# svohr/mixemt

Hardware: AMD Instinct MI355X
Metric: read x hap cells/sec through the EM iteration (EM iters/sec reported beside it as em_iters_per_s), 1000000 reads x 5408 haps in total, whole job (higher is better)
Workload: dtype f64

## Files before the change

include/mixemt_hip_tuning.h:

```cpp
#ifndef MIXEMT_HIP_TUNING_H
#define MIXEMT_HIP_TUNING_H

#include <stddef.h>
#include <stdint.h>

#ifdef __cplusplus
extern "C" {
#endif

struct mxm_em_state;

int mxm_reset_tuning(void);

int mxm_set_timing_events(void *ev_start, void *ev_stop);

int mxm_describe_stream_kernel(int32_t H, int32_t nb, char *buf, size_t len);

int mxm_diag_stream_read(const void *src, size_t bytes, int32_t wg_per_cu, int32_t blocked,
                         void *sink, void *stream);

struct mxm_coded;
int mxm_diag_stream_coded(const struct mxm_coded *c, int32_t H, int32_t wg_per_cu, void *sink, void *stream);

int mxm_diag_stream_quads(const struct mxm_coded *c, int32_t H, int32_t wg_per_cu, void *sink, void *stream);

int mxm_set_progress_callback(void (*fn)(const struct mxm_em_state *state_host, int32_t B, void *user),
                              void *user, int32_t every);

int mxm_set_loop_graph(int32_t mode);

int mxm_set_loop_fused(int32_t mode, int32_t chunk);

int mxm_set_fused_coded_grid(int32_t nwg);

int mxm_set_quad_left_grid(int32_t nwg);

int mxm_set_sparse_long_rows(int32_t on);
int mxm_set_sparse_long_entries(int32_t n);

int mxm_set_quad_encoder(int32_t kind);

int mxm_set_coded_batch_tile(int32_t bt);

int mxm_diag_fused_force_abort(int32_t on);

int mxm_diag_fused_stamps(const void *ws, unsigned long long *out_host);

int mxm_set_batch_tile(int32_t bt);

int mxm_set_compact_restarts(int32_t mode);

#define MXM_SAMPLES_TILE_ROWS 32
int mxm_samples_tile_rows(void);

int mxm_set_min_rows_per_wg(int32_t n);

int mxm_set_sparse_max_distinct(int32_t n);

#ifdef __cplusplus
}
#endif
#endif
```

mixemt_amd/_lib.py:

```python

import ctypes
import os

_PKG = os.path.dirname(os.path.abspath(__file__))
LIB_PATH = os.environ.get("MXM_LIB") or os.path.join(_PKG, "lib", "libmixemt_hip.so")

c_i32, c_i64, c_f64 = ctypes.c_int32, ctypes.c_int64, ctypes.c_double
c_ptr, c_size = ctypes.c_void_p, ctypes.c_size_t


class EmState(ctypes.Structure):
    _fields_ = [("done", c_i32), ("iters", c_i32), ("l1", c_f64), ("ticket", ctypes.c_uint32), ("error", ctypes.c_uint32)]


class Coded(ctypes.Structure):
    _fields_ = [("rec", c_ptr), ("rec_off", c_ptr), ("ndist", c_ptr), ("R", c_i64),
                ("P_rest", c_ptr), ("ldp_rest", c_i64), ("w_rest", c_ptr), ("R_rest", c_i64),
                ("wide_rows", c_ptr), ("n_wide", c_i64),
                ("qrec", c_ptr), ("qoff", c_ptr), ("nquad", c_ptr), ("quad_rows", c_ptr), ("n_quad_rows", c_i64),
                ("byte_rows", c_ptr), ("n_byte_rows", c_i64)]


class SampleTile(ctypes.Structure):
    _fields_ = [("sample", c_i32), ("count", c_i32), ("first", c_i64)]
# ... 80 lines not shown
                                         ctypes.POINTER(EmState)]),
    "mxm_samples_tile_rows": (ctypes.c_int, []),
    "mxm_samples_plan": (c_i64, [c_ptr, c_i32, c_ptr, c_i64, c_ptr]),
    "mxm_samples_workspace_bytes": (c_size, [c_i64, c_i32, c_i32]),
    "mxm_em_iter_samples": (ctypes.c_int, [ctypes.POINTER(Coded), c_ptr, c_i32, c_ptr, c_ptr, c_i32, c_ptr, c_ptr, c_ptr,
                                           c_size, c_ptr]),
    "mxm_em_loop_samples": (ctypes.c_int, [ctypes.POINTER(Coded), c_ptr, c_i32, c_ptr, c_i32, c_ptr, c_ptr, c_ptr, c_ptr,
                                           c_ptr, c_f64, c_i32, c_i32, c_ptr, c_size, c_ptr, ctypes.POINTER(EmState)]),
    "mxm_em_step": (ctypes.c_int, [c_ptr, c_i64, c_ptr, c_ptr, c_i64, c_i32, c_ptr, c_i64, c_i32,
                                   c_ptr, c_ptr, c_size, c_ptr]),
    "mxm_log_normalize": (ctypes.c_int, [c_ptr, c_i32, c_ptr, c_ptr]),
    "mxm_l1_exp_diff": (ctypes.c_int, [c_ptr, c_ptr, c_i32, c_ptr, c_ptr]),
    "mxm_add_scalar": (ctypes.c_int, [c_ptr, c_i64, c_i64, c_i32, c_f64, c_ptr]),
    "mxm_assign_reads": (ctypes.c_int, [c_ptr, c_i64, c_ptr, c_ptr, c_i32, c_i64, c_i32, c_f64, c_ptr, c_ptr]),
    "mxm_diag_stream_read": (ctypes.c_int, [c_ptr, c_size, c_i32, c_i32, c_ptr, c_ptr]),
    "mxm_diag_stream_coded": (ctypes.c_int, [ctypes.POINTER(Coded), c_i32, c_i32, c_ptr, c_ptr]),
    "mxm_diag_stream_quads": (ctypes.c_int, [ctypes.POINTER(Coded), c_i32, c_i32, c_ptr, c_ptr]),
    "mxm_diag_fused_force_abort": (ctypes.c_int, [c_i32]),
    "mxm_set_fused_coded_grid": (ctypes.c_int, [c_i32]),
    "mxm_set_quad_left_grid": (ctypes.c_int, [c_i32]),
    "mxm_set_coded_batch_tile": (ctypes.c_int, [c_i32]),
    "mxm_set_sparse_long_rows": (ctypes.c_int, [c_i32]),
    "mxm_set_quad_encoder": (ctypes.c_int, [c_i32]),
    "mxm_set_sparse_long_entries": (ctypes.c_int, [c_i32]),
    "mxm_diag_fused_stamps": (ctypes.c_int, [c_ptr, ctypes.POINTER(ctypes.c_ulonglong)]),
    "mxm_set_timing_events": (ctypes.c_int, [c_ptr, c_ptr]),
    "mxm_set_batch_tile": (ctypes.c_int, [c_i32]),
    "mxm_encode_signatures": (ctypes.c_int64, [ctypes.c_char_p, c_ptr, c_i64, c_ptr, c_i64, c_ptr, c_ptr, c_ptr,
                                               c_i64]),
    "mxm_aln_encode": (ctypes.c_int, [ctypes.POINTER(AlnColumns), c_ptr, c_i64, c_ptr, c_i32, c_i32, c_i32, c_i32,
                                      ctypes.POINTER(c_ptr)]),
    "mxm_aln_sizes_of": (ctypes.c_int, [c_ptr, ctypes.POINTER(AlnSizes)]),
    "mxm_aln_fetch": (ctypes.c_int, [c_ptr, c_ptr, c_ptr, c_ptr, c_ptr, c_ptr, c_ptr, c_ptr, c_ptr, c_ptr]),
    "mxm_aln_fetch_fragments": (ctypes.c_int, [c_ptr, c_ptr, c_ptr, c_ptr, c_ptr]),
    "mxm_aln_free": (None, [c_ptr]),
    "mxm_bam_read": (ctypes.c_int, [ctypes.c_char_p, c_i32, ctypes.POINTER(c_ptr)]),
    "mxm_bam_sizes_of": (ctypes.c_int, [c_ptr, ctypes.POINTER(BamSizes)]),
    "mxm_bam_columns": (ctypes.c_int, [c_ptr, ctypes.POINTER(AlnColumns)]),
    "mxm_bam_fetch_names": (ctypes.c_int, [c_ptr, c_ptr, c_ptr, c_ptr, c_ptr]),
    "mxm_bam_free": (None, [c_ptr]),
    "mxm_observe_bases": (ctypes.c_int, [ctypes.POINTER(AlnColumns), c_ptr, c_i32, c_i32, c_i64, c_ptr, c_ptr]),
    "mxm_observe_bases_labelled": (ctypes.c_int, [ctypes.POINTER(AlnColumns), c_ptr, c_ptr, c_i32, c_i32, c_i32, c_i64,
                                                  c_ptr, c_ptr]),
    "mxm_consensus": (ctypes.c_int, [c_ptr, c_i32, c_i64, c_i64, c_i64, c_i32, c_ptr, c_ptr, c_ptr, c_ptr]),
    "mxm_new_variants": (ctypes.c_int, [c_ptr, c_i64, c_i32, ctypes.POINTER(c_i32), c_i32, c_i64, c_ptr, c_ptr, c_ptr]),
    "mxm_first_observed": (ctypes.c_int, [ctypes.POINTER(AlnColumns), c_ptr, c_ptr, c_i32, c_i32, c_i32, c_i64, c_ptr,
                                          c_ptr, c_ptr]),
    "mxm_extend_assign": (ctypes.c_int, [ctypes.POINTER(AlnColumns), c_ptr, c_ptr, c_i32, c_i32, ctypes.POINTER(c_i32),
                                         c_i32, c_i32, c_i32, c_i32, c_ptr, c_i64, c_ptr, c_ptr, c_ptr, c_ptr]),
    "mxm_set_compact_restarts": (ctypes.c_int, [c_i32]),
    "mxm_set_loop_graph": (ctypes.c_int, [c_i32]),
    "mxm_set_loop_fused": (ctypes.c_int, [c_i32, c_i32]),
    "mxm_set_progress_callback": (ctypes.c_int, [c_ptr, c_ptr, c_i32]),
    "mxm_set_min_rows_per_wg": (ctypes.c_int, [c_i32]),
    "mxm_reset_tuning": (ctypes.c_int, []),
    "mxm_describe_stream_kernel": (ctypes.c_int, [c_i32, c_i32, ctypes.c_char_p, c_size]),
    "mxm_set_sparse_max_distinct": (ctypes.c_int, [c_i32]),
    "mxm_row_argmax_votes": (ctypes.c_int, [c_ptr, c_i64, c_ptr, c_i64, c_i32, c_ptr, c_ptr,
                                            c_ptr, c_size, c_ptr]),
    "mxm_first_seen": (ctypes.c_int, [c_ptr, c_i64, c_i32, c_ptr, c_ptr]),
    "mxm_gather_columns": (ctypes.c_int, [c_ptr, c_i64, c_i64, c_i32, c_ptr, c_i32, c_ptr, c_i64, c_ptr]),
    "mxm_fold_logaddexp": (ctypes.c_int, [c_ptr, c_i64, ctypes.POINTER(c_ptr), ctypes.POINTER(c_i64), c_i32,
                                          c_i64, c_i32, c_f64, c_ptr]),
}

FINISH_SIGNATURES = {
    "mxm_samples_finish_workspace_bytes": (c_size, [c_i64, c_i32, c_i32]),
    "mxm_votes_samples": (ctypes.c_int, [ctypes.POINTER(Coded), c_ptr, c_i32, c_i32, c_ptr, c_ptr, c_ptr, c_ptr, c_ptr, c_ptr,
                                         c_ptr, c_ptr, c_ptr, c_ptr, c_ptr, c_size, c_ptr]),
    "mxm_gather_columns_samples": (ctypes.c_int, [ctypes.POINTER(Coded), c_ptr, c_i32, c_i32, c_ptr, c_ptr, c_i32, c_ptr,
                                                  c_ptr, c_size, c_ptr]),
    "mxm_em_loop_samples_narrow": (ctypes.c_int, [ctypes.POINTER(Coded), c_ptr, c_i32, c_i32, c_ptr, c_i32, c_ptr, c_ptr,
                                                  c_ptr, c_ptr, c_ptr, c_ptr, c_f64, c_i32, c_i32, c_ptr, c_ptr, c_size,
                                                  c_ptr, ctypes.POINTER(EmState)]),
    "mxm_assign_reads_samples": (ctypes.c_int, [ctypes.POINTER(Coded), c_ptr, c_i32, c_i32, c_ptr, c_i32, c_ptr, c_ptr,
                                                c_ptr, c_ptr, c_ptr, c_ptr, c_f64, c_ptr, c_ptr, c_ptr, c_size, c_ptr]),
}

VARCHECK_SIGNATURES = {
    "mxm_check_variants_samples": (ctypes.c_int, [c_ptr, c_i32, c_i64, c_ptr, c_ptr, c_i32, c_ptr, c_ptr, c_i32, c_i64, c_ptr,
                                                  c_ptr, c_i32, c_f64, c_f64, c_f64, c_i32, c_i32, c_ptr, c_ptr, c_ptr, c_ptr]),
}

ABI_VERSION = 603

PROGRESS_FN = ctypes.CFUNCTYPE(None, ctypes.POINTER(EmState), c_i32, c_ptr)

_lib = None


class MixemtHipError(RuntimeError):
    pass


def load():
    global _lib
    if _lib is not None:
        return _lib
    if not os.path.exists(LIB_PATH):
        raise MixemtHipError(
            "libmixemt_hip.so is not built (%s); run `python -m mixemt_amd.build` -- "
            "there is no CPU fallback for the EM hot path" % LIB_PATH)
    from . import _dev
    lib = ctypes.CDLL(LIB_PATH)
    try:
        lib.mxm_version.restype = ctypes.c_int
        lib.mxm_version.argtypes = []
        have = lib.mxm_version()
    except AttributeError:
        have = None
    if have != ABI_VERSION:
        raise MixemtHipError("%s reports ABI version %s, this binding was written for %d: rebuild with "
                             "`python -m mixemt_amd.build --force`" % (LIB_PATH, have, ABI_VERSION))
    for name, (restype, argtypes) in (list(SIGNATURES.items()) + list(FINISH_SIGNATURES.items())
                                      + list(VARCHECK_SIGNATURES.items())):
        try:
            fn = getattr(lib, name)
        except AttributeError:
            raise MixemtHipError("%s has ABI version %d but lacks %s: rebuild with "
                                 "`python -m mixemt_amd.build --force`" % (LIB_PATH, have, name))
        fn.restype = restype
        fn.argtypes = argtypes
    _lib = lib
    try:
        if _dev.torch is not None and _dev.torch.cuda.is_available():
            lib.mxm_preload()
    except Exception:
        pass
    return lib


def check(rc, what):
    if rc != 0:
        msg = load().mxm_last_error().decode("utf-8", "replace")
        raise ValueError("%s failed (%d): %s" % (what, rc, msg))
```

mixemt_amd/build.py:

```python

import hashlib
import os
import shutil
import subprocess
import sys

_PKG = os.path.dirname(os.path.abspath(__file__))
_ROOT = os.path.dirname(_PKG)
SRC = os.path.join(_PKG, "csrc", "mixemt_hip.hip")
HDRS = [os.path.join(_ROOT, "include", name) for name in ("mixemt_hip.h", "mixemt_hip_tuning.h", "mixemt_hip_samples_finish.h",
                                                           "mixemt_hip_var_check.h")]
LIB_DIR = os.path.join(_PKG, "lib")
LIB = os.path.join(LIB_DIR, "libmixemt_hip.so")
ARCH = "gfx950"


def _hipcc():
    for cand in (os.environ.get("HIPCC"), shutil.which("hipcc"), "/opt/rocm/bin/hipcc"):
        if cand and os.path.exists(cand):
            return cand
    raise RuntimeError("hipcc not found (set HIPCC or add /opt/rocm/bin to PATH)")


def _sources():
    csrc = os.path.dirname(SRC)
    return sorted(os.path.join(csrc, f) for f in os.listdir(csrc) if f.endswith((".hip", ".hpp"))) + HDRS


def _digest(flags):
    h = hashlib.sha256()
    for path in _sources():
        with open(path, "rb") as fin:
            h.update(fin.read())
    h.update(" ".join(flags).encode())
    return h.hexdigest()


def build(force=False, defines=(), verbose=False, out=None):
    global LIB
    if out is not None:
        LIB = os.path.abspath(out)
    flags = ["--offload-arch=%s" % ARCH, "-O3", "-std=c++17", "-shared", "-fPIC", "-Werror=format",
             "-I" + os.path.join(_ROOT, "include"), "-I" + os.path.dirname(SRC)]
    flags += ["-D%s" % d for d in defines]
    stamp = LIB + ".stamp"
    want = _digest(flags)
    if not force and os.path.exists(LIB) and os.path.exists(stamp):
        with open(stamp) as fin:
            if fin.read().strip() == want:
                return LIB
    os.makedirs(os.path.dirname(LIB), exist_ok=True)
    cmd = [_hipcc()] + flags + [SRC, "-o", LIB, "-lz"]
    if verbose:
        sys.stderr.write(" ".join(cmd) + "\n")
    proc = subprocess.run(cmd, stdout=subprocess.PIPE, stderr=subprocess.STDOUT, text=True)
    if proc.returncode != 0:
        raise RuntimeError("hipcc failed:\n" + proc.stdout)
    with open(stamp, "w") as fout:
        fout.write(want + "\n")
    return LIB


if __name__ == "__main__":
    defs = []
    argv = sys.argv[1:]
    i = 0
    while i < len(argv):
        if argv[i] == "-D":
            defs.append(argv[i + 1])
            i += 2
        elif argv[i].startswith("-D"):
            defs.append(argv[i][2:])
            i += 1
        else:
            i += 1
    out_path = argv[argv.index("--out") + 1] if "--out" in argv else None
    print(build(force="--force" in argv, defines=defs, verbose=True, out=out_path))
```

mixemt_amd/csrc/coded_kernels.hpp:

```cpp
#ifndef MIXEMT_CODED_KERNELS_HPP
#define MIXEMT_CODED_KERNELS_HPP

#define ENC_THREADS 256
#define ENC_SLOTS 1024
#define ENC_MAX_CODES 256
#define ENC_MAX_WIDE 1024
#define ENC_WIDE_SLOTS 4096
#define ENC_EMPTY 0xFFFFFFFFFFFFFFFFull

__host__ __device__ __forceinline__ int rec_code_bytes(int nd, int ldc) { return nd > ENC_MAX_CODES ? 2 * ldc : ldc; }
__device__ __forceinline__ int rec_code_at(const uint8_t *codes, int h, bool wide) {
    return wide ? (int)reinterpret_cast<const uint16_t *>(codes)[h] : (int)codes[h];
}

template <int NCH, bool WIDE>
__device__ __forceinline__ void encode_one_row(int64_t r, const double *__restrict__ M, int64_t ldm, int H, int ldc,
                                               uint8_t *__restrict__ rec, int64_t rec_cap, int64_t *__restrict__ rec_off,
                                               int32_t *__restrict__ ndist, double *__restrict__ rowmax,
                                               unsigned long long *__restrict__ stats) {
    constexpr int NW = ENC_THREADS / 64;
    constexpr int SLOTS = WIDE ? ENC_WIDE_SLOTS : ENC_SLOTS;
    constexpr int MAXC = WIDE ? ENC_MAX_WIDE : ENC_MAX_CODES;
    constexpr int SPT = SLOTS / ENC_THREADS;
    __shared__ unsigned long long s_key[SLOTS];
// ... 89 lines not shown
            }
        }
    }
    __syncthreads();
    const bool dense = (s_flag != 0);

    int cnt = 0;
#pragma unroll
    for (int j = 0; j < SPT; ++j) cnt += (s_key[SPT * t + j] != ENC_EMPTY) ? 1 : 0;
    const int incl = wave_inclusive_scan_i32(cnt);
    if (lane == 63) s_wcnt[wv] = incl;
    __syncthreads();
    int base = 0, D = 0;
#pragma unroll
    for (int q = 0; q < NW; ++q) {
        if (q < wv) base += s_wcnt[q];
        D += s_wcnt[q];
    }
    const int cbytes = WIDE ? 2 * ldc : ldc;
    const int64_t bytes = (int64_t)cbytes + 16 * (int64_t)D;
    const bool coded = !dense && D <= MAXC && (!WIDE || D > ENC_MAX_CODES);
    if (t == 0) {
        long long off = -1;
        if (coded) {
            off = (long long)atomicAdd(&stats[0], (unsigned long long)bytes);
            if (off + bytes > rec_cap) off = -1;
        }
        s_off = off;
    }
    int code = base + incl - cnt;
#pragma unroll
    for (int j = 0; j < SPT; ++j) {
        if (s_key[SPT * t + j] != ENC_EMPTY) s_code[SPT * t + j] = (unsigned short)code++;
    }
    __syncthreads();
    const long long off = s_off;
    if (off >= 0) {
        double *tbl = reinterpret_cast<double *>(rec + off + cbytes);
        code = base + incl - cnt;
#pragma unroll
        for (int j = 0; j < SPT; ++j) {
            const unsigned long long kk = s_key[SPT * t + j];
            if (kk != ENC_EMPTY) {
                const double mval = __longlong_as_double((long long)kk);
                tbl[code] = exp(mval - shift);
                tbl[D + code] = mval;
                ++code;
            }
        }
#pragma unroll
        for (int k = 0; k < NCH; ++k) {
            const int c0 = 4 * (t + k * ENC_THREADS);
            if (c0 < ldc) {
                unsigned int cd[4];
#pragma unroll
                for (int e = 0; e < 4; ++e) cd[e] = (c0 + e < H) ? (unsigned int)s_code[slot[k][e]] : 0u;
                if constexpr (WIDE) {
                    u2 word;
                    word.x = cd[0] | (cd[1] << 16);
                    word.y = cd[2] | (cd[3] << 16);
                    reinterpret_cast<u2 *>(rec + off)[t + k * ENC_THREADS] = word;
                } else {
                    reinterpret_cast<unsigned int *>(rec + off)[t + k * ENC_THREADS] =
                        cd[0] | (cd[1] << 8) | (cd[2] << 16) | (cd[3] << 24);
                }
            }
        }
    }
    if (t == 0) {
        if constexpr (WIDE) {
            if (off >= 0) {
                ndist[r] = D;
                rec_off[r] = off;
                atomicAdd(&stats[1], ~0ull);
            }
        } else {
            rowmax[r] = shift;
            ndist[r] = (off >= 0) ? D : 0;
            rec_off[r] = (off >= 0) ? off : 0;
            if (off < 0) atomicAdd(&stats[1], 1ull);
        }
    }
    __syncthreads();
}

template <int NCH>
__global__ __launch_bounds__(ENC_THREADS) void encode_rows_kernel(
    const double *__restrict__ M, int64_t ldm, int64_t R, int H, int ldc, uint8_t *__restrict__ rec, int64_t rec_cap,
    int64_t *__restrict__ rec_off, int32_t *__restrict__ ndist, double *__restrict__ rowmax,
    unsigned long long *__restrict__ stats) {
    for (int64_t r = blockIdx.x; r < R; r += gridDim.x)
        encode_one_row<NCH, false>(r, M, ldm, H, ldc, rec, rec_cap, rec_off, ndist, rowmax, stats);
}

template <int NCH>
__global__ __launch_bounds__(ENC_THREADS) void encode_wide_rows_kernel(
    const double *__restrict__ M, int64_t ldm, int64_t R, int H, int ldc, uint8_t *__restrict__ rec, int64_t rec_cap,
    int64_t *__restrict__ rec_off, int32_t *__restrict__ ndist, double *__restrict__ rowmax,
    unsigned long long *__restrict__ stats) {
    constexpr int CH = 32;
    __shared__ int s_list[CH];
    __shared__ int s_nlist;
    const int t = threadIdx.x;
    const int64_t nchunk = (R + CH - 1) / CH;
    for (int64_t c = blockIdx.x; c < nchunk; c += gridDim.x) {
        if (t == 0) s_nlist = 0;
        __syncthreads();
        const int64_t r = c * CH + t;
        if (t < CH && r < R && ndist[r] == 0) s_list[atomicAdd(&s_nlist, 1)] = t;
        __syncthreads();
        const int n = s_nlist;
        for (int i = 0; i < n; ++i)
            encode_one_row<NCH, true>(c * CH + s_list[i], M, ldm, H, ldc, rec, rec_cap, rec_off, ndist, rowmax, stats);
        __syncthreads();
    }
}

template <int THREADS, int NCH, int NBUF, bool NT, bool RESIDENT, bool WIDE_PREFETCH, bool CHECK = false>
__device__ __forceinline__ void coded_row_pass(const uint8_t *__restrict__ rec, const int64_t *__restrict__ rec_off,
                                               const int32_t *__restrict__ ndist, int ldc, const double *__restrict__ w,
                                               const int64_t *__restrict__ wide_rows, int64_t n_wide, int64_t R,
                                               const double (&p)[NCH][4], double (&acc)[NCH][4], bool &meta_ready,
                                               int *chk_result = nullptr, const int64_t *__restrict__ row_list = nullptr,
                                               int64_t n_list = 0, const int32_t *__restrict__ nquad = nullptr, int vbid = -1,
                                               int vgrid = 0) {
    static_assert(NBUF >= 3, "codes NBUF - 1 rows ahead, tables NBUF - 2");
    constexpr int NW = THREADS / 64;
    constexpr int AUX = NT ? 2 : 0;
    __shared__ double s_tbl[NBUF][ENC_MAX_CODES];
    __shared__ __attribute__((aligned(16))) double red[NBUF][NW];
    const int t = threadIdx.x, lane = t & 63, wv = t >> 6;
    const int nword = ldc >> 2;
    const int64_t bid = vbid >= 0 ? (int64_t)vbid : (int64_t)blockIdx.x, grid = vbid >= 0 ? (int64_t)vgrid : (int64_t)gridDim.x;
    const row_deal deal(row_list != nullptr ? n_list : R, bid, grid);
    const int voff = t * 4;
    int last_w = t + (NCH - 1) * THREADS;
    if (last_w > nword - 1) last_w = nword - 1;
    const int voff_last = last_w * 4;
    const bool tbl_thread = (THREADS <= ENC_MAX_CODES) || t < ENC_MAX_CODES;
    const int tslot = t & (ENC_MAX_CODES - 1);
    typedef unsigned int u2v __attribute__((ext_vector_type(2)));
    __shared__ int s_chk[2];
    if constexpr (CHECK) {
        if (t == 0) s_chk[0] = s_chk[1] = 0;
        __syncthreads();
    }
    auto list_row = [&](int64_t e) -> int64_t {
        int64_t r = wide_rows[e];
        if constexpr (CHECK) {
            if (r < 0 || r >= R || (e > 0 && wide_rows[e - 1] >= r)) {
                s_chk[1] = 1;
                r = -1;
            }
        }
        return r;
    };
    auto list_nd = [&](int64_t r) -> int {
        if (r < 0) return 0;
        int nd = ndist[r];
        if constexpr (CHECK) {
            if (nd <= ENC_MAX_CODES) {
                s_chk[1] = 1;
                nd = 0;
            }
        }
        return nd;
// ... 444 lines not shown
```

mixemt_amd/csrc/mixemt_hip.hip:

```cpp
#include <hip/hip_runtime.h>
#include <stdint.h>
#include <stdio.h>
#include <stdlib.h>
#include <string.h>
#include <math.h>
#include <algorithm>
#include <atomic>
#include <mutex>
#include <type_traits>
#include <utility>
#include <vector>

#include "mixemt_hip.h"
#include "mixemt_hip_tuning.h"

#include "common.hpp"
#include "aln_encode.hpp"
#include "bam_reader.hpp"
#include "coded_kernels.hpp"
#include "quad_kernels.hpp"
#include "quad_batched_kernels.hpp"
#include "build_kernels.hpp"
#include "build_lut_kernels.hpp"
#include "build_sparse_kernels.hpp"
#include "em_kernels.hpp"
#include "estep_kernels.hpp"
#include "aux_kernels.hpp"
#include "records_kernels.hpp"
#include "fused_kernels.hpp"
#include "fused_cols_kernels.hpp"
#include "fused_coded_kernels.hpp"
#include "fused_narrow_kernels.hpp"
#include "samples_kernels.hpp"
#include "samples_finish_kernels.hpp"
#include "exchange.hpp"
#include "aln_walk.hpp"
#include "observe_kernels.hpp"
#include "var_check_kernels.hpp"
#include "assemble_kernels.hpp"


struct mxm_em_state;
typedef void (*mxm_progress_fn)(const mxm_em_state *state_host, int32_t B, void *user);
struct mxm_tuning {
    int sparse_maxd = -1;
    int min_rows_per_wg = 8;
    int compact_restarts = 2;
    int max_bt = 4;
    int loop_graph = -1;
    int loop_fused = -1;
    int fused_chunk = 0;
    int fused_cols = 1;
    int fused_coded_wg = 0;
    int quad_left_wg = 0;
    int sparse_long_entries = 5120;
    int quad_encoder = 1;
    int sparse_long = 1;
    int coded_bt = 3;
    int fused_force_abort = 0;
    double fused_cells = 1.0e8;
    hipEvent_t ev_start = nullptr, ev_stop = nullptr;
    mxm_progress_fn progress = nullptr;
    void *progress_user = nullptr;
    int progress_every = 10;
};
static std::mutex g_tune_mu;
static mxm_tuning g_tune;
static thread_local mxm_tuning T;
#define MXM_ENTER() do { std::lock_guard<std::mutex> lk_(g_tune_mu); T = g_tune; } while (0)
template <typename F>
static int tune_set(F f) {
    std::lock_guard<std::mutex> lk(g_tune_mu);
    f(g_tune);
    return 0;
}
extern "C" int mxm_reset_tuning(void) {
    return tune_set([](mxm_tuning &t) { t = mxm_tuning(); });
}

static inline int clamp_grid(int64_t want, int cap) {
    if (want < 1) want = 1;
    return (int)(want < cap ? want : cap);
}

static inline int64_t part_ld(int H) { return ((int64_t)H + 1) & ~(int64_t)1; }

static hipError_t raise_dynamic_lds(const void *kernel, size_t bytes, const char *name) {
    const hipError_t e = hipFuncSetAttribute(kernel, hipFuncAttributeMaxDynamicSharedMemorySize, (int)bytes);
    if (e != hipSuccess)
        snprintf(g_err, sizeof(g_err), "%s: cannot opt into %zu bytes of dynamic LDS: %s", name, bytes,
                 hipGetErrorString(e));
    return e;
}
static int dynamic_lds_ok(const void *kernel, size_t bytes, const char *name, const char *who = nullptr, int H = 0,
                          const char *too_wide = nullptr) {
    if (too_wide != nullptr && bytes > 150 * 1024) return fail(-1, "%s: H=%d %s", who, H, too_wide);
    if (bytes > 60 * 1024 && raise_dynamic_lds(kernel, bytes, name) != hipSuccess) return -2;
    return 0;
}

#define RC_TRY(expr)                                                                         \
    do {                                                                                     \
        const int rc_ = (expr);                                                              \
        if (rc_ != 0) return rc_;                                                            \
    } while (0)

template <int MAX, typename F>
static bool dispatch_width(int n, F &&f) {
    if constexpr (MAX < 1) {
        return false;
    } else {
        if (n != MAX) return dispatch_width<MAX - 1>(n, f);
        f(std::integral_constant<int, MAX>{});
        return true;
    }
}

extern "C" int mxm_version(void) { return MXM_VERSION; }
extern "C" const char *mxm_last_error(void) { return g_err; }

extern "C" int mxm_linear_supported(int32_t H) {
    return (H >= MXM_LINEAR_MIN_H && H <= 8192) ? 1 : 0;
}

static size_t fused_sync_bytes() { return (sizeof(fused_sync) + 255) & ~(size_t)255; }
static size_t fused_snapshot_bytes(int H, int B) {
    return ((size_t)3 * B * H * sizeof(double) + (size_t)B * sizeof(mxm_em_state) + 255) & ~(size_t)255;
}
static size_t fused_rows_bytes(int H, int nwg) { return (size_t)(nwg + 2) * part_ld(H) * sizeof(double); }
static size_t fused_cols_bytes(int64_t R, int nwg) {
    const size_t ldz = (size_t)((R + 1) & ~(int64_t)1);
    return ((size_t)(nwg + 1) * ldz + 2 * (size_t)nwg) * sizeof(double);
}

extern "C" size_t mxm_workspace_bytes(int64_t R, int32_t H, int32_t B) {
    const size_t tiles = (size_t)MXM_MAX_WG * MXM_MAX_BT * (size_t)part_ld(H) * sizeof(double);
    size_t fused = fused_rows_bytes(H, MXM_MAX_WG);
    if (R > 0 && R <= (int64_t)FCOLS_MAX_RPT * FCOLS_THREADS) fused = std::max(fused, fused_cols_bytes(R, MXM_MAX_WG));
    fused += fused_sync_bytes() + fused_snapshot_bytes(H, B > 0 ? B : 1) + 512;
// ... 226 lines not shown
        rec_off == nullptr || ndist == nullptr || rowmax == nullptr || stats == nullptr)
        return fail(-1, "mxm_build_em_records: record buffer (16-byte aligned, >= one record) and output arrays required");
    spb_records out;
    out.rec = rec;
    out.rec_cap = (long long)rec_bytes;
    out.rec_off = rec_off;
    out.ndist = ndist;
    out.rowmax = rowmax;
    out.stats = reinterpret_cast<unsigned long long *>(stats);
    out.ldc = coded_ld(H);
    return build_sparse_impl("mxm_build_em_records", maj, lhit, lmiss, mk_ptr, mk_hap, mk_base, row_ptr, site, obs, order,
                             R, H, S, M, ldm, &out, fallback, n_fallback, (hipStream_t)stream);
}

template <typename ST>
static int linearize_wide(const double *M, int64_t ldm, int64_t R, int H, ST *P, int64_t ldp, double *rowmax,
                          hipStream_t s) {
    const int nch = (H / 2 + 255) / 256;
    int cap = num_cu() * 2 < MXM_MAX_WG ? num_cu() * 2 : MXM_MAX_WG;
    const int nwg = clamp_grid((R + 1) / 2, cap);
    const bool ok = dispatch_width<16>(nch, [&](auto n) {
        hipLaunchKernelGGL((linearize_wide_kernel<decltype(n)::value, ST>), dim3(nwg), dim3(256), 0, s, M, ldm, R, H, P, ldp, rowmax);
    });
    return ok ? 0 : 1;
}

static inline bool wide_rows_ok(const void *M, int64_t ldm, int H) {
    return ((H & 1) == 0) && ((ldm & 1) == 0) && ((reinterpret_cast<uintptr_t>(M) & 15) == 0) && H >= 64 && H <= 8192;
}

extern "C" int mxm_linearize(const double *M, int64_t ldm, int64_t R, int32_t H, double *P, int64_t ldp,
                             double *rowmax, void *stream) {
    if (R < 0 || H <= 0) return fail(-1, "mxm_linearize: bad shape");
    if (ldm < H || ldp < H || (ldp & 1)) return fail(-1, "mxm_linearize: ldp must be even and >= H (ldp=%lld)", (long long)ldp);
    if (R == 0) return 0;
    if (wide_rows_ok(M, ldm, H) && (reinterpret_cast<uintptr_t>(P) & 15) == 0 &&
        linearize_wide<double>(M, ldm, R, (int)H, P, ldp, rowmax, (hipStream_t)stream) == 0) {
        HIP_TRY(hipGetLastError());
        return 0;
    }
    const int grid = clamp_grid(R, num_cu() * 8);
    hipLaunchKernelGGL(linearize_kernel, dim3(grid), dim3(ROW_THREADS), 0, (hipStream_t)stream, M, ldm, R,
                       (int)H, P, ldp, rowmax);
    HIP_TRY(hipGetLastError());
    return 0;
}

extern "C" int mxm_set_timing_events(void *ev_start, void *ev_stop) {
    return tune_set([=](mxm_tuning &t) { t.ev_start = (hipEvent_t)ev_start; t.ev_stop = (hipEvent_t)ev_stop; });
}

extern "C" int mxm_set_min_rows_per_wg(int32_t n) {
    if (n < 1) return fail(-1, "mxm_set_min_rows_per_wg: n < 1");
    return tune_set([n](mxm_tuning &t) { t.min_rows_per_wg = n; });
}

extern "C" int mxm_set_compact_restarts(int32_t mode) {
    return tune_set([mode](mxm_tuning &t) { t.compact_restarts = mode < 0 ? 0 : (mode > 2 ? 2 : mode); });
}

extern "C" int mxm_set_batch_tile(int32_t bt) {
    if (bt < 1 || bt > 4) return fail(-1, "mxm_set_batch_tile: tile must be 1..4");
    return tune_set([bt](mxm_tuning &t) { t.max_bt = bt; });
}

extern "C" int mxm_set_fused_coded_grid(int32_t nwg) {
    return tune_set([nwg](mxm_tuning &t) { t.fused_coded_wg = nwg > 0 ? nwg : 0; });
}

extern "C" int mxm_set_sparse_long_rows(int32_t on) {
    return tune_set([on](mxm_tuning &t) { t.sparse_long = on ? 1 : 0; });
}
extern "C" int mxm_set_sparse_long_entries(int32_t n) {
    return tune_set([n](mxm_tuning &t) { t.sparse_long_entries = n > 0 ? n : 0; });
}
extern "C" int mxm_set_coded_batch_tile(int32_t bt) {
    if (bt != 1 && bt != 3) return fail(-1, "mxm_set_coded_batch_tile: 1 or 3, got %d", bt);
    return tune_set([bt](mxm_tuning &t) { t.coded_bt = bt; });
}
extern "C" int mxm_set_quad_encoder(int32_t kind) {
    if (kind != 0 && kind != 1) return fail(-1, "mxm_set_quad_encoder: 0 or 1, got %d", kind);
    return tune_set([kind](mxm_tuning &t) { t.quad_encoder = kind; });
}
extern "C" int mxm_set_quad_left_grid(int32_t nwg) {
    return tune_set([nwg](mxm_tuning &t) { t.quad_left_wg = nwg > 0 ? nwg : 0; });
}

extern "C" int mxm_diag_fused_force_abort(int32_t on) {
    return tune_set([on](mxm_tuning &t) { t.fused_force_abort = on ? 1 : 0; });
}

#ifndef MXM_V1_THREADS
#define MXM_V1_THREADS 256
#endif
#ifndef MXM_V1_NBUF
#define MXM_V1_NBUF 2
#endif
#ifndef MXM_V1_WG_PER_CU
#define MXM_V1_WG_PER_CU 2
#endif
#ifndef MXM_V2_THREADS
#define MXM_V2_THREADS 512
#endif
#ifndef MXM_V2_NBUF
#define MXM_V2_NBUF 2
#endif
#ifndef MXM_V3_THREADS
#define MXM_V3_THREADS 512
#endif
#ifndef MXM_V3_NBUF
#define MXM_V3_NBUF 2
#endif
#ifndef MXM_V4_THREADS
#define MXM_V4_THREADS 512
#endif
#ifndef MXM_V4_NBUF
#define MXM_V4_NBUF 2
#endif
#ifndef MXM_V2_PREG
#define MXM_V2_PREG 1
#endif
#ifndef MXM_V3_PREG
#define MXM_V3_PREG 2
#endif
#ifndef MXM_V4_PREG
#define MXM_V4_PREG 2
#endif
#ifndef MXM_V1B_THREADS
#define MXM_V1B_THREADS 512
#endif
#ifndef MXM_V1B_NBUF
#define MXM_V1B_NBUF 3
#endif
#define MXM_MAX_COL2 4096
#define MXM_LDS_BUDGET (156 * 1024)

static inline int variant_threads(int nb) {
    return nb == 1 ? MXM_V1_THREADS : (nb == 2 ? MXM_V2_THREADS : (nb == 3 ? MXM_V3_THREADS : MXM_V4_THREADS));
}
static inline int variant_preg(int nb) {
    return nb == 1 ? 1 : (nb == 2 ? MXM_V2_PREG : (nb == 3 ? MXM_V3_PREG : MXM_V4_PREG));
}

static size_t batch_lds_bytes(int H, int nb) {
    const int threads = variant_threads(nb);
    const int nch = ((H + 1) / 2 + threads - 1) / threads;
    return (size_t)(nb - variant_preg(nb)) * nch * threads * 16;
}

static bool batch_fits(int H, int nb) {
    if (nb <= 1) return true;
    static const int max_nch[MXM_MAX_BT + 1] = {0, 16, 8, 7, 6};
    const int threads = variant_threads(nb);
    const int nch = ((H + 1) / 2 + threads - 1) / threads;
    return nch <= max_nch[nb] && batch_lds_bytes(H, nb) <= MXM_LDS_BUDGET;
}

template <int THREADS, int NCH, int BT, int NBUF, int PREG>
static int launch_wide(const double *P, int64_t ldp, const double *w, const double *props, int64_t R,
                       int H, int grid, double *partial, int64_t ldpart,
                       const mxm_em_state *state, mxm_slots slots, hipStream_t stream) {
    if constexpr (NCH * THREADS > MXM_MAX_COL2) {
        return fail(-1, "mxm_em_iter: H=%d outside the linear kernel's range", H);
    } else {
        const size_t lds = (size_t)(BT - PREG) * NCH * THREADS * sizeof(d2);
        RC_TRY(dynamic_lds_ok(reinterpret_cast<const void *>(&em_iter_wide_kernel<THREADS, NCH, BT, NBUF, PREG>), lds, "em_iter_wide_kernel"));
// ... 180 lines not shown
        hipLaunchKernelGGL((estep_global_kernel<true>), dim3(nwg), dim3(ROW_THREADS), 0, stream, M, ldm, w, ln_props, R, H,
                           (double *)nullptr, (int64_t)0, 0, partial, ldpart, state, (const int64_t *)nullptr);
        HIP_TRY(hipGetLastError());
    } else if (H <= MXM_NARROW_MAX_H) {
        const int rc = launch_narrow<true>(M, ldm, w, ln_props, R, H, (double *)nullptr, (int64_t)0, 0, partial, ldpart,
                                           state, stream, &nwg);
        if (rc != 0) return rc;
    } else {
        nwg = clamp_grid(R, num_cu() * 2 < MXM_MAX_WG ? num_cu() * 2 : MXM_MAX_WG);
        RC_TRY(dynamic_lds_ok(reinterpret_cast<const void *>(&estep_log_kernel<true>), lds, "estep_log_kernel"));
        hipLaunchKernelGGL((estep_log_kernel<true>), dim3(nwg), dim3(ROW_THREADS), lds, stream, M, ldm, w, ln_props,
                           R, H, (double *)nullptr, (int64_t)0, 0, partial, ldpart, state);
        HIP_TRY(hipGetLastError());
    }
    return reduce_one(partial, nwg, H, colsum, state, stream);
}

extern "C" int mxm_em_iter(const double *M, int64_t ldm, const double *P, int64_t ldp, const double *w,
                           const double *props, const double *ln_props, int64_t R, int32_t H, int32_t B,
                           const mxm_em_state *state, double *colsum, void *ws, size_t ws_bytes, void *stream) {
    MXM_ENTER();
    if (R <= 0 || H <= 0 || B <= 0) return fail(-1, "mxm_em_iter: bad shape R=%lld H=%d", (long long)R, H);
    if (ws == nullptr || ws_bytes < mxm_workspace_bytes(R, H, B)) return fail(-1, "mxm_em_iter: workspace too small");
    if (P != nullptr && ((ldp & 1) || ldp < H)) return fail(-1, "mxm_em_iter: ldp must be even and >= H");
    if (M != nullptr && ldm < H) return fail(-1, "mxm_em_iter: ldm < H");
    const bool linear = (P != nullptr) && mxm_linear_supported(H);
    int max_bt = linear ? T.max_bt : 1;
    while (max_bt > 1 && !batch_fits((int)H, max_bt)) --max_bt;
    for (int b = 0; b < B;) {
        const int left = B - b;
        const int passes = (left + max_bt - 1) / max_bt;
        const int nb = (left + passes - 1) / passes;
        const mxm_em_state *st = state ? state + b : nullptr;
        int rc;
        if (linear)
            rc = em_iter_linear_tile(P, ldp, w, props, R, (int)H, nb, slots_from(b), state, colsum, (double *)ws,
                                     (hipStream_t)stream, b == 0);
        else
            rc = em_iter_log_one(M, ldm, w, ln_props ? ln_props + (int64_t)b * H : nullptr, R, (int)H, st,
                                 colsum + (int64_t)b * H, (double *)ws, (hipStream_t)stream);
        if (rc != 0) return rc;
        b += nb;
    }
    return 0;
}

extern "C" int mxm_linearize_f32(const double *M, int64_t ldm, int64_t R, int32_t H, float *P, int64_t ldp,
                                 double *rowmax, void *stream) {
    if (R < 0 || H <= 0) return fail(-1, "mxm_linearize_f32: bad shape");
    if (ldm < H || ldp < H || (ldp & 3)) return fail(-1, "mxm_linearize_f32: ldp must be a multiple of 4 and >= H (ldp=%lld)", (long long)ldp);
    if (R == 0) return 0;
    if (wide_rows_ok(M, ldm, H) && (reinterpret_cast<uintptr_t>(P) & 7) == 0 && (ldp & 1) == 0 &&
        linearize_wide<float>(M, ldm, R, (int)H, P, ldp, rowmax, (hipStream_t)stream) == 0) {
        HIP_TRY(hipGetLastError());
        return 0;
    }
    const int grid = clamp_grid(R, num_cu() * 8);
    hipLaunchKernelGGL(linearize_f32_kernel, dim3(grid), dim3(ROW_THREADS), 0, (hipStream_t)stream, M, ldm, R, (int)H,
                       P, ldp, rowmax);
    HIP_TRY(hipGetLastError());
    return 0;
}

extern "C" int mxm_em_iter_f32(const float *P, int64_t ldp, const double *w, const double *props, int64_t R,
                               int32_t H, int32_t B, const mxm_em_state *state, double *colsum, void *ws,
                               size_t ws_bytes, void *stream) {
    MXM_ENTER();
    if (R <= 0 || H <= 0 || B <= 0) return fail(-1, "mxm_em_iter_f32: bad shape R=%lld H=%d", (long long)R, H);
    if (!mxm_linear_supported(H)) return fail(-1, "mxm_em_iter_f32: H=%d outside the linear kernel's range", H);
    if (P == nullptr || (ldp & 3) || ldp < H) return fail(-1, "mxm_em_iter_f32: ldp must be a multiple of 4 and >= H");
    if (ws == nullptr || ws_bytes < mxm_workspace_bytes(R, H, B)) return fail(-1, "mxm_em_iter_f32: workspace too small");
    for (int b = 0; b < B; ++b) {
        const int rc = em_iter_f32_one(P, ldp, w, props + (int64_t)b * H, R, (int)H, state ? state + b : nullptr,
                                       colsum + (int64_t)b * H, (double *)ws, (hipStream_t)stream, b == 0);
        if (rc != 0) return rc;
    }
    return 0;
}

extern "C" size_t mxm_coded_bytes(int64_t R, int32_t H) { return mxm_record_bytes(R, H); }

extern "C" int mxm_encode_rows(const double *M, int64_t ldm, int64_t R, int32_t H, uint8_t *rec, size_t rec_bytes,
                               int64_t *rec_off, int32_t *ndist, double *rowmax, int64_t *stats, void *stream) {
    if (R <= 0 || H <= 0 || ldm < H) return fail(-1, "mxm_encode_rows: bad shape R=%lld H=%d", (long long)R, H);
    if (!mxm_linear_supported(H) || (reinterpret_cast<uintptr_t>(M) & 7) != 0)
        return fail(-1, "mxm_encode_rows: needs H in [65, 8192] (H=%d ldm=%lld)", H, (long long)ldm);
    if (rec == nullptr || (reinterpret_cast<uintptr_t>(rec) & 15) || rec_bytes < (size_t)coded_ld(H) + 16 * ENC_MAX_CODES)
        return fail(-1, "mxm_encode_rows: record buffer missing, unaligned or smaller than one record");
    if (rec_off == nullptr || ndist == nullptr || rowmax == nullptr || stats == nullptr)
        return fail(-1, "mxm_encode_rows: output arrays required");
    hipStream_t s = (hipStream_t)stream;
    HIP_TRY(hipMemsetAsync(stats, 0, 2 * sizeof(int64_t), s));
    const int ldc = coded_ld(H);
    const int nch = (ldc / 4 + ENC_THREADS - 1) / ENC_THREADS;
    const int grid = clamp_grid(R, num_cu() * 4);
    const int grid_w = clamp_grid((R + 31) / 32, num_cu() * 3);
    const bool ok = dispatch_width<8>(nch, [&](auto n) {
        constexpr int NCH = decltype(n)::value;
        unsigned long long *st = reinterpret_cast<unsigned long long *>(stats);
        hipLaunchKernelGGL((encode_rows_kernel<NCH>), dim3(grid), dim3(ENC_THREADS), 0, s, M, ldm, R, (int)H, ldc, rec,
                           (int64_t)rec_bytes, rec_off, ndist, rowmax, st);
        hipLaunchKernelGGL((encode_wide_rows_kernel<NCH>), dim3(grid_w), dim3(ENC_THREADS), 0, s, M, ldm, R, (int)H, ldc, rec,
                           (int64_t)rec_bytes, rec_off, ndist, rowmax, st);
    });
    if (!ok) return fail(-1, "mxm_encode_rows: H=%d outside the kernel's range", H);
    HIP_TRY(hipGetLastError());
    return 0;
}

static int coded_check(const mxm_coded *c, int32_t H, const char *who) {
    if (c == nullptr || c->R <= 0 || H <= 0 || !mxm_linear_supported(H))
        return fail(-1, "%s: bad coded matrix (rows %lld, H %d)", who, (long long)(c ? c->R : 0), H);
    if (c->rec == nullptr || c->rec_off == nullptr || c->ndist == nullptr) return fail(-1, "%s: coded matrix arrays missing", who);
    if (c->R_rest < 0 || (c->R_rest > 0 && (c->P_rest == nullptr || c->ldp_rest < H || (c->ldp_rest & 1) ||
                                            (reinterpret_cast<uintptr_t>(c->P_rest) & 15))))
        return fail(-1, "%s: the dense rest needs 16-byte aligned rows with an even ld >= H", who);
    if (c->n_wide < 0 || (c->n_wide > 0 && c->wide_rows == nullptr)) return fail(-1, "%s: n_wide > 0 needs wide_rows", who);
    if (c->qrec != nullptr) {
        if (c->qoff == nullptr || c->nquad == nullptr || c->n_quad_rows < 0 || c->n_byte_rows < 0 ||
            (c->n_quad_rows > 0 && c->quad_rows == nullptr) || (c->n_byte_rows > 0 && c->byte_rows == nullptr) ||
            (reinterpret_cast<uintptr_t>(c->qrec) & 31))
            return fail(-1, "%s: quad dictionary arrays missing (or qrec not 32-byte aligned)", who);
        if (c->n_quad_rows + c->n_byte_rows + c->n_wide + c->R_rest != c->R)
            return fail(-1, "%s: quad_rows + byte_rows + wide_rows + the dense rest must be all %lld rows", who, (long long)c->R);
    }
    return 0;
}

static int rest_check(const char *who, int32_t H, const double *M_rest, int64_t ldm_rest, const int64_t *rest_rows, int64_t n_rest) {
    if (n_rest < 0 || (n_rest > 0 && (M_rest == nullptr || rest_rows == nullptr || ldm_rest < H)))
        return fail(-1, "%s: the rows without a record need M_rest, rest_rows and ldm_rest >= H", who);
    return 0;
}

extern "C" size_t mxm_quad_bytes(int64_t R, int32_t H) {
    (void)H;
    constexpr size_t largest = QUAD_CODE_BYTES + QUAD_MAX * 32, per_piece = (size_t)QUAD_CHUNK / largest;
    return R > 0 ? (((size_t)R + per_piece - 1) / per_piece + 5120) * (size_t)QUAD_CHUNK : 0;
}

extern "C" int mxm_expand_tables(const uint8_t *maj, const int32_t *mk_ptr, const uint16_t *mk_hap, const uint8_t *mk_base,
                                 const uint8_t *map256, int32_t S, int32_t H, int64_t lde, uint8_t *out, void *stream) {
    if (maj == nullptr || mk_ptr == nullptr || mk_hap == nullptr || mk_base == nullptr || out == nullptr || S <= 0 || H <= 0 || lde < H)
        return fail(-1, "mxm_expand_tables: bad arguments");
    hipLaunchKernelGGL(expand_tables_kernel, dim3(clamp_grid(S, num_cu() * 8)), dim3(256), 0, (hipStream_t)stream, maj, mk_ptr, mk_hap,
                       mk_base, map256, (int)S, (int)H, lde, out);
    HIP_TRY(hipGetLastError());
    return 0;
}

extern "C" size_t mxm_quad_lists_scratch_bytes(int64_t R) {
    return R > 0 ? (size_t)((R + QLIST_CHUNK - 1) / QLIST_CHUNK) * 2 * sizeof(long long) : 0;
}

extern "C" int mxm_quad_lists(const int32_t *ndist, const int32_t *nquad, int64_t R, int64_t *quad_rows, int64_t *byte_rows,
                              int64_t *counts, void *scratch, size_t scratch_bytes, void *stream) {
    MXM_ENTER();
    if (ndist == nullptr || nquad == nullptr || R <= 0 || quad_rows == nullptr || byte_rows == nullptr || counts == nullptr)
        return fail(-1, "mxm_quad_lists: bad arguments");
    if (scratch == nullptr || scratch_bytes < mxm_quad_lists_scratch_bytes(R)) return fail(-1, "mxm_quad_lists: scratch too small");
    const int64_t nchunk = (R + QLIST_CHUNK - 1) / QLIST_CHUNK;
    if (nchunk > 0x7fffffff) return fail(-1, "mxm_quad_lists: too many rows");
    hipStream_t s = (hipStream_t)stream;
    long long *cc = static_cast<long long *>(scratch);
    hipLaunchKernelGGL(quad_list_count_kernel, dim3((unsigned)nchunk), dim3(QLIST_THREADS), 0, s, ndist, nquad, R, cc);
    hipLaunchKernelGGL(quad_list_scan_kernel, dim3(1), dim3(QLIST_THREADS), 0, s, cc, nchunk, reinterpret_cast<long long *>(counts));
    hipLaunchKernelGGL(quad_list_fill_kernel, dim3((unsigned)nchunk), dim3(QLIST_THREADS), 0, s, ndist, nquad, R, cc, quad_rows, byte_rows);
    HIP_TRY(hipGetLastError());
    return 0;
}

extern "C" int mxm_build_quads(const mxm_coded *c, int32_t H, uint8_t *qrec, size_t qrec_bytes, int64_t *qoff, int32_t *nquad,
                               uint64_t *stats, void *stream) {
    MXM_ENTER();
    if (c == nullptr || c->R <= 0 || c->rec == nullptr || c->rec_off == nullptr || c->ndist == nullptr || !mxm_linear_supported(H))
        return fail(-1, "mxm_build_quads: bad coded matrix (rows %lld, H %d)", (long long)(c ? c->R : 0), H);
    if (qoff == nullptr || nquad == nullptr || stats == nullptr || (qrec == nullptr && qrec_bytes > 0) ||
        (reinterpret_cast<uintptr_t>(qrec) & 31))
        return fail(-1, "mxm_build_quads: qoff, nquad, stats and a 32-byte aligned qrec required");
    const int ldc = coded_ld(H);
    if (ldc / 4 > 8 * QUAD_THREADS) return fail(-1, "mxm_build_quads: H=%d beyond eight quads per thread", H);
    HIP_TRY(hipMemsetAsync(stats, 0, 2 * sizeof(uint64_t), (hipStream_t)stream));
    if (T.quad_encoder == 1 && ldc / 4 <= 64 * QW_K)
        hipLaunchKernelGGL(quad_encode_wave_kernel, dim3(clamp_grid((c->R + QW_WAVES - 1) / QW_WAVES, std::min(num_cu() * QW_MIN_WAVES, 5120 / QW_WAVES))), dim3(QUAD_THREADS),
                           0, (hipStream_t)stream, c->rec, c->rec_off, c->ndist, ldc, (int)H, c->R, qrec,
                           (unsigned long long)qrec_bytes, qoff, nquad, reinterpret_cast<unsigned long long *>(stats));
// ... 1685 lines not shown
```

Baseline: 867.6 billion.

## Add list-based row encoder with occupancy-list ranking and double-buffered flags

Adds new row-encoding kernels that record the occupied hash slots in a small list. For rows with few distinct values, codes are assigned by a single-wave rank over that list instead of scanning the whole hash table. Parity-indexed flags and counters drop some barriers between the rows a block processes, and runs of equal values reuse the previous slot to skip hash probes. The new encoder is on by default through a tuning knob. It targets encode preprocessing cost, at the price of more code and the risk of subtle races when buffers are reused across parity slots.

```diff
diff --git a/include/mixemt_hip_row_encoder.h b/include/mixemt_hip_row_encoder.h
--- /dev/null
+++ b/include/mixemt_hip_row_encoder.h
@@ -0,0 +1,14 @@
+#ifndef MIXEMT_HIP_ROW_ENCODER_H
+#define MIXEMT_HIP_ROW_ENCODER_H
+
+#ifdef __cplusplus
+extern "C" {
+#endif
+
+int mxm_set_row_encoder(int32_t kind);
+
+#ifdef __cplusplus
+}
+#endif
+
+#endif
diff --git a/include/mixemt_hip_tuning.h b/include/mixemt_hip_tuning.h
--- a/include/mixemt_hip_tuning.h
+++ b/include/mixemt_hip_tuning.h
@@ -60,4 +60,7 @@
 #ifdef __cplusplus
 }
 #endif
+
+#include "mixemt_hip_row_encoder.h"
+
 #endif
diff --git a/mixemt_amd/_lib.py b/mixemt_amd/_lib.py
--- a/mixemt_amd/_lib.py
+++ b/mixemt_amd/_lib.py
@@ -186,6 +186,10 @@
                                                   c_ptr, c_i32, c_f64, c_f64, c_f64, c_i32, c_i32, c_ptr, c_ptr, c_ptr, c_ptr]),
 }
 
+ENCODER_SIGNATURES = {
+    "mxm_set_row_encoder": (ctypes.c_int, [c_i32]),
+}
+
 ABI_VERSION = 603
 
 PROGRESS_FN = ctypes.CFUNCTYPE(None, ctypes.POINTER(EmState), c_i32, c_ptr)
@@ -217,7 +221,7 @@
         raise MixemtHipError("%s reports ABI version %s, this binding was written for %d: rebuild with "
                              "`python -m mixemt_amd.build --force`" % (LIB_PATH, have, ABI_VERSION))
     for name, (restype, argtypes) in (list(SIGNATURES.items()) + list(FINISH_SIGNATURES.items())
-                                      + list(VARCHECK_SIGNATURES.items())):
+                                      + list(VARCHECK_SIGNATURES.items()) + list(ENCODER_SIGNATURES.items())):
         try:
             fn = getattr(lib, name)
         except AttributeError:
diff --git a/mixemt_amd/build.py b/mixemt_amd/build.py
--- a/mixemt_amd/build.py
+++ b/mixemt_amd/build.py
@@ -9,7 +9,7 @@
 _ROOT = os.path.dirname(_PKG)
 SRC = os.path.join(_PKG, "csrc", "mixemt_hip.hip")
 HDRS = [os.path.join(_ROOT, "include", name) for name in ("mixemt_hip.h", "mixemt_hip_tuning.h", "mixemt_hip_samples_finish.h",
-                                                           "mixemt_hip_var_check.h")]
+                                                           "mixemt_hip_var_check.h", "mixemt_hip_row_encoder.h")]
 LIB_DIR = os.path.join(_PKG, "lib")
 LIB = os.path.join(LIB_DIR, "libmixemt_hip.so")
 ARCH = "gfx950"
diff --git a/mixemt_amd/csrc/coded_kernels.hpp b/mixemt_amd/csrc/coded_kernels.hpp
--- a/mixemt_amd/csrc/coded_kernels.hpp
+++ b/mixemt_amd/csrc/coded_kernels.hpp
@@ -195,6 +195,291 @@
         }
     }
     __syncthreads();
+}
+
+template <int NCH, bool WIDE>
+__device__ __forceinline__ void encode_one_row_list(int64_t r, int it, const double *__restrict__ M, int64_t ldm, int H, int ldc,
+                                                    uint8_t *__restrict__ rec, int64_t rec_cap, int64_t *__restrict__ rec_off,
+                                                    int32_t *__restrict__ ndist, double *__restrict__ rowmax,
+                                                    unsigned long long *__restrict__ stats) {
+    constexpr int NW = ENC_THREADS / 64;
+    constexpr int SLOTS = WIDE ? ENC_WIDE_SLOTS : ENC_SLOTS;
+    constexpr int MAXC = WIDE ? ENC_MAX_WIDE : ENC_MAX_CODES;
+    constexpr int SPT = SLOTS / ENC_THREADS;
+    constexpr int RANK_MAX = 64;
+    __shared__ unsigned long long s_key[SLOTS];
+    __shared__ unsigned short s_code[SLOTS];
+    __shared__ unsigned short s_occ[WIDE ? 1 : MAXC];
+    __shared__ double s_red[NW];
+    __shared__ int s_wcnt[NW];
+    __shared__ int s_flag[2], s_n[2];
+    __shared__ long long s_off;
+    const int t = threadIdx.x, lane = t & 63, wv = __builtin_amdgcn_readfirstlane(t >> 6);
+    const int par = it & 1;
+    typedef unsigned int u4 __attribute__((ext_vector_type(4)));
+    typedef unsigned int u2 __attribute__((ext_vector_type(2)));
+
+    if (it == 0) {
+#pragma unroll
+        for (int q = 0; q < SPT; ++q) s_key[t + q * ENC_THREADS] = ENC_EMPTY;
+        if (t < 2) {
+            s_flag[t] = 0;
+            s_n[t] = 0;
+        }
+        __syncthreads();
+    }
+
+    const auto rsrc = __builtin_amdgcn_make_buffer_rsrc(const_cast<double *>(M + r * ldm), 0, H * 8, 0x00020000);
+    double x[NCH][4];
+#pragma unroll
+    for (int k = 0; k < NCH; ++k) {
+        const int off = (t + k * ENC_THREADS) * 32;
+        const d2 a = __builtin_bit_cast(d2, (u4)__builtin_amdgcn_raw_buffer_load_b128(rsrc, off, 0, 2));
+        const d2 b = __builtin_bit_cast(d2, (u4)__builtin_amdgcn_raw_buffer_load_b128(rsrc, off, 16, 2));
+        x[k][0] = a.x;
+        x[k][1] = a.y;
+        x[k][2] = b.x;
+        x[k][3] = b.y;
+    }
+    if (H & 1) {
+        const double tail = M[r * ldm + (H - 1)];
+#pragma unroll
+        for (int k = 0; k < NCH; ++k) {
+            if (4 * (t + k * ENC_THREADS) == H - 1) x[k][0] = tail;
+            if (4 * (t + k * ENC_THREADS) + 2 == H - 1) x[k][2] = tail;
+        }
+    }
+    double m = -INFINITY;
+#pragma unroll
+    for (int k = 0; k < NCH; ++k)
+#pragma unroll
+        for (int e = 0; e < 4; ++e)
+            if (4 * (t + k * ENC_THREADS) + e < H) m = fmax(m, x[k][e]);
+    m = wave_max(m);
+    if (lane == 0) s_red[wv] = m;
+    int slot[NCH][4];
+    unsigned long long prev_key = ENC_EMPTY;
+    int prev_slot = 0;
+#pragma unroll
+    for (int k = 0; k < NCH; ++k) {
+        const bool give_up = *(volatile int *)&s_flag[par] != 0;
+#pragma unroll
+        for (int e = 0; e < 4; ++e) {
+            const bool valid = 4 * (t + k * ENC_THREADS) + e < H;
+            const unsigned long long key = (unsigned long long)__double_as_longlong(x[k][e]);
+            int sl = 0;
+            bool need = valid;
+            if (valid && key == ENC_EMPTY) {
+                s_flag[par] = 1;
+                need = false;
+            }
+            if (need && key == prev_key) {
+                sl = prev_slot;
+                need = false;
+            }
+            if (give_up) need = false;
+            if (need) {
+                unsigned int h = (unsigned int)((key ^ (key >> 29)) * 0x9E3779B97F4A7C15ull >> 40) & (SLOTS - 1);
+                for (int probes = 0;; ++probes) {
+                    const unsigned long long old = atomicCAS(&s_key[h], ENC_EMPTY, key);
+                    if (old == ENC_EMPTY) {
+                        const int idx = atomicAdd(&s_n[par], 1);
+                        if (idx >= MAXC) s_flag[par] = 1;
+                        else if constexpr (!WIDE) s_occ[idx] = (unsigned short)h;
+                        break;
+                    }
+                    if (old == key) break;
+                    h = (h + 1) & (SLOTS - 1);
+                    if (probes >= SLOTS) {
+                        s_flag[par] = 1;
+                        break;
+                    }
+                }
+                sl = (int)h;
+            }
+            slot[k][e] = sl;
+            if (valid) {
+                prev_key = key;
+                prev_slot = sl;
+            }
+        }
+    }
+    __syncthreads();
+    const bool dense = __builtin_amdgcn_readfirstlane(s_flag[par]) != 0;
+    const int nocc =__builtin_amdgcn_readfirstlane(s_n[par]);
+    m = fmax(fmax(s_red[0], s_red[1]), fmax(s_red[2], s_red[3]));
+    const double shift = isfinite(m) ? m : 0.0;
+    const int cbytes = WIDE ? 2 * ldc : ldc;
+
+    auto write_codes = [&](long long off) {
+        int last_slot = -1;
+        unsigned int last_code = 0;
+#pragma unroll
+        for (int k = 0; k < NCH; ++k) {
+            const int c0 = 4 * (t + k * ENC_THREADS);
+            if (c0 < ldc) {
+                unsigned int cd[4];
+#pragma unroll
+                for (int e = 0; e < 4; ++e) {
+                    cd[e] = 0u;
+                    if (c0 + e < H) {
+                        if (WIDE || slot[k][e] != last_slot) {
+                            last_slot = slot[k][e];
+                            last_code = (unsigned int)s_code[last_slot];
+                        }
+                        cd[e] = last_code;
+                    }
+                }
+                if constexpr (WIDE) {
+                    u2 word;
+                    word.x = cd[0] | (cd[1] << 16);
+                    word.y = cd[2] | (cd[3] << 16);
+                    reinterpret_cast<u2 *>(rec + off)[t + k * ENC_THREADS] = word;
+                } else {
+                    reinterpret_cast<unsigned int *>(rec + off)[t + k * ENC_THREADS] =
+                        cd[0] | (cd[1] << 8) | (cd[2] << 16) | (cd[3] << 24);
+                }
+            }
+        }
+    };
+    auto write_meta = [&](long long off, int D) {
+        if constexpr (WIDE) {
+            if (off >= 0) {
+                ndist[r] = D;
+                rec_off[r] = off;
+                atomicAdd(&stats[1], ~0ull);
+            }
+        } else {
+            rowmax[r] = shift;
+            ndist[r] = (off >= 0) ? D : 0;
+            rec_off[r] = (off >= 0) ? off : 0;
+            if (off < 0) atomicAdd(&stats[1], 1ull);
+        }
+    };
+    auto allocate = [&](int64_t bytes) -> long long {
+        long long off = (long long)atomicAdd(&stats[0], (unsigned long long)bytes);
+        if (off + bytes > rec_cap) off = -1;
+        return off;
+    };
+
+    if constexpr (!WIDE) {
+        if (!dense && nocc <= RANK_MAX) {
+            const int D = nocc;
+            int my = 0x7fffffff, rank = 0;
+            unsigned long long kk = 0;
+            if (wv == 0) {
+                long long off0 = 0;
+                if (t == 0) off0 = allocate((int64_t)cbytes + 16 * (int64_t)D);
+                if (lane < D) {
+                    my = (int)s_occ[lane];
+                    kk = s_key[my];
+                }
+                for (int j = 0; j < D; ++j) rank += (__builtin_amdgcn_readlane(my, j) < my) ? 1 : 0;
+                if (lane < D) {
+                    s_code[my] = (unsigned short)rank;
+                    s_key[my] = ENC_EMPTY;
+                }
+                if (t == 0) s_off = off0;
+            }
+            __syncthreads();
+            const long long off = s_off;
+            if (off >= 0) {
+                if (lane < D && wv == 0) {
+                    double *tbl = reinterpret_cast<double *>(rec + off + cbytes);
+                    const double mval = __longlong_as_double((long long)kk);
+                    tbl[rank] = exp(mval - shift);
+                    tbl[D + rank] = mval;
+                }
+                write_codes(off);
+            }
+            if (t == 0) {
+                write_meta(off, D);
+                s_n[par] = 0;
+            }
+            return;
+        }
+    }
+
+    int cnt = 0;
+#pragma unroll
+    for (int j = 0; j < SPT; ++j) cnt += (s_key[SPT * t + j] != ENC_EMPTY) ? 1 : 0;
+    const int incl = wave_inclusive_scan_i32(cnt);
+    if (lane == 63) s_wcnt[wv] = incl;
+    __syncthreads();
+    int base = 0, D = 0;
+#pragma unroll
+    for (int q = 0; q < NW; ++q) {
+        if (q < wv) base += s_wcnt[q];
+        D += s_wcnt[q];
+    }
+    const bool coded = !dense && D <= MAXC && (!WIDE || D > ENC_MAX_CODES);
+    if (t == 0) {
+        s_off = coded ? allocate((int64_t)cbytes + 16 * (int64_t)D) : -1;
+        s_flag[par] = 0;
+        s_n[par] = 0;
+    }
+    int code = base + incl - cnt;
+#pragma unroll
+    for (int j = 0; j < SPT; ++j) {
+        if (s_key[SPT * t + j] != ENC_EMPTY) s_code[SPT * t + j] = (unsigned short)code++;
+    }
+    __syncthreads();
+    const long long off = s_off;
+    if (off >= 0) {
+        double *tbl = reinterpret_cast<double *>(rec + off + cbytes);
+        code = base + incl - cnt;
+#pragma unroll
+        for (int j = 0; j < SPT; ++j) {
+            const unsigned long long kk = s_key[SPT * t + j];
+            if (kk != ENC_EMPTY) {
+                const double mval = __longlong_as_double((long long)kk);
+                tbl[code] = exp(mval - shift);
+                tbl[D + code] = mval;
+                ++code;
+                s_key[SPT * t + j] = ENC_EMPTY;
+            }
+        }
+        write_codes(off);
+    } else {
+#pragma unroll
+        for (int j = 0; j < SPT; ++j) s_key[SPT * t + j] = ENC_EMPTY;
+    }
+    if (t == 0) write_meta(off, D);
+    __syncthreads();
+}
+
+template <int NCH>
+__global__ __launch_bounds__(ENC_THREADS) void encode_rows_list_kernel(
+    const double *__restrict__ M, int64_t ldm, int64_t R, int H, int ldc, uint8_t *__restrict__ rec, int64_t rec_cap,
+    int64_t *__restrict__ rec_off, int32_t *__restrict__ ndist, double *__restrict__ rowmax,
+    unsigned long long *__restrict__ stats) {
+    int it = 0;
+    for (int64_t r = blockIdx.x; r < R; r += gridDim.x, ++it)
+        encode_one_row_list<NCH, false>(r, it, M, ldm, H, ldc, rec, rec_cap, rec_off, ndist, rowmax, stats);
+}
+
+template <int NCH>
+__global__ __launch_bounds__(ENC_THREADS) void encode_wide_rows_list_kernel(
+    const double *__restrict__ M, int64_t ldm, int64_t R, int H, int ldc, uint8_t *__restrict__ rec, int64_t rec_cap,
+    int64_t *__restrict__ rec_off, int32_t *__restrict__ ndist, double *__restrict__ rowmax,
+    unsigned long long *__restrict__ stats) {
+    constexpr int CH = 32;
+    __shared__ int s_rows[CH];
+    __shared__ int s_nrows;
+    const int t = threadIdx.x;
+    const int64_t nchunk = (R + CH - 1) / CH;
+    int it = 0;
+    for (int64_t c = blockIdx.x; c < nchunk; c += gridDim.x) {
+        if (t == 0) s_nrows = 0;
+        __syncthreads();
+        const int64_t r = c * CH + t;
+        if (t < CH && r < R && ndist[r] == 0) s_rows[atomicAdd(&s_nrows, 1)] = t;
+        __syncthreads();
+        const int n = s_nrows;
+        for (int i = 0; i < n; ++i, ++it)
+            encode_one_row_list<NCH, true>(c * CH + s_rows[i], it, M, ldm, H, ldc, rec, rec_cap, rec_off, ndist, rowmax, stats);
+        __syncthreads();
+    }
 }
 
 template <int NCH>
diff --git a/mixemt_amd/csrc/mixemt_hip.hip b/mixemt_amd/csrc/mixemt_hip.hip
--- a/mixemt_amd/csrc/mixemt_hip.hip
+++ b/mixemt_amd/csrc/mixemt_hip.hip
@@ -55,6 +55,7 @@
     int quad_left_wg = 0;
     int sparse_long_entries = 5120;
     int quad_encoder = 1;
+    int row_encoder = 1;
     int sparse_long = 1;
     int coded_bt = 3;
     int fused_force_abort = 0;
@@ -447,6 +448,10 @@
     if (kind != 0 && kind != 1) return fail(-1, "mxm_set_quad_encoder: 0 or 1, got %d", kind);
     return tune_set([kind](mxm_tuning &t) { t.quad_encoder = kind; });
 }
+extern "C" int mxm_set_row_encoder(int32_t kind) {
+    if (kind != 0 && kind != 1) return fail(-1, "mxm_set_row_encoder: 0 or 1, got %d", kind);
+    return tune_set([kind](mxm_tuning &t) { t.row_encoder = kind; });
+}
 extern "C" int mxm_set_quad_left_grid(int32_t nwg) {
     return tune_set([nwg](mxm_tuning &t) { t.quad_left_wg = nwg > 0 ? nwg : 0; });
 }
@@ -793,6 +798,7 @@
 
 extern "C" int mxm_encode_rows(const double *M, int64_t ldm, int64_t R, int32_t H, uint8_t *rec, size_t rec_bytes,
                                int64_t *rec_off, int32_t *ndist, double *rowmax, int64_t *stats, void *stream) {
+    MXM_ENTER();
     if (R <= 0 || H <= 0 || ldm < H) return fail(-1, "mxm_encode_rows: bad shape R=%lld H=%d", (long long)R, H);
     if (!mxm_linear_supported(H) || (reinterpret_cast<uintptr_t>(M) & 7) != 0)
         return fail(-1, "mxm_encode_rows: needs H in [65, 8192] (H=%d ldm=%lld)", H, (long long)ldm);
@@ -809,10 +815,12 @@
     const bool ok = dispatch_width<8>(nch, [&](auto n) {
         constexpr int NCH = decltype(n)::value;
         unsigned long long *st = reinterpret_cast<unsigned long long *>(stats);
-        hipLaunchKernelGGL((encode_rows_kernel<NCH>), dim3(grid), dim3(ENC_THREADS), 0, s, M, ldm, R, (int)H, ldc, rec,
-                           (int64_t)rec_bytes, rec_off, ndist, rowmax, st);
-        hipLaunchKernelGGL((encode_wide_rows_kernel<NCH>), dim3(grid_w), dim3(ENC_THREADS), 0, s, M, ldm, R, (int)H, ldc, rec,
-                           (int64_t)rec_bytes, rec_off, ndist, rowmax, st);
+        const auto first = T.row_encoder == 1 ? encode_rows_list_kernel<NCH> : encode_rows_kernel<NCH>;
+        const auto second = T.row_encoder == 1 ? encode_wide_rows_list_kernel<NCH> : encode_wide_rows_kernel<NCH>;
+        hipLaunchKernelGGL(first, dim3(grid), dim3(ENC_THREADS), 0, s, M, ldm, R, (int)H, ldc, rec, (int64_t)rec_bytes, rec_off,
+                           ndist, rowmax, st);
+        hipLaunchKernelGGL(second, dim3(grid_w), dim3(ENC_THREADS), 0, s, M, ldm, R, (int)H, ldc, rec, (int64_t)rec_bytes, rec_off,
+                           ndist, rowmax, st);
     });
     if (!ok) return fail(-1, "mxm_encode_rows: H=%d outside the kernel's range", H);
     HIP_TRY(hipGetLastError());
```

Result: no change. 866.0 billion (-0.2%).
